# Zhongxu-Wang/ArtSpeech

Hardware: AMD Instinct MI355X
Metric: mel frames/sec (whole job; per-GPU = value / n_gpus), acoustic-model inference path, batch 32 x 200-frame utterances (higher is better)
Workload: dtype f32 (f16x3 split-operand MFMA, fp32 accumulate)

## Files before the change

### artspeech_amd/csrc/elementwise.hip

```cpp
#include "common.h"
#include <algorithm>
#include <cstring>
#include "artspeech_hip.h"
#include "conv_gemm.h"
#define AS_FILE_CLS AS_CLS_OTHER

static __device__ __forceinline__ float wave_sum(float v)
{
#pragma unroll
    for (int o = 32; o > 0; o >>= 1) v += __shfl_xor(v, o);
    return v;
}

static __device__ __forceinline__ float lrelu02(float v) { return v > 0.f ? v : 0.2f * v; }

__global__ void make_meta_kernel(const int* __restrict__ widths, const int* __restrict__ col_off, int B, int H,
                                 unsigned long long* __restrict__ meta, unsigned* __restrict__ status)
{
    const int b = blockIdx.y;
    const int W = widths[b];
    const int base = col_off[b];
    if (W > AS_META_MAX_W) {
        if (blockIdx.x == 0 && threadIdx.x == 0) as_status_raise(status, AS_STATUS_BAD_LAYOUT);
        return;
// ... 359 lines not shown
        return AS_EINVAL;
    if (N == 0) return AS_OK;
    const size_t wsz = (size_t)MM * K * sizeof(float);
    AsProfScope prof__(AS_FILE_CLS, 2.0 * M * K * (double)N, 4.0 * (K + M) * (double)N, s);
    const dim3 grid(as_cdiv(N, 64)), block(256);
    if (M == 1) hipLaunchKernelGGL(project_cols_kernel<1>, grid, block, wsz, s, x, ldx, K, N, w, bias, M, y, ldy, pros, ld_pros, col_off, B, track0);
    else if (M <= 4) hipLaunchKernelGGL(project_cols_kernel<4>, grid, block, wsz, s, x, ldx, K, N, w, bias, M, y, ldy, pros, ld_pros, col_off, B, track0);
    else hipLaunchKernelGGL(project_cols_kernel<16>, grid, block, wsz, s, x, ldx, K, N, w, bias, M, y, ldy, pros, ld_pros, col_off, B, track0);
    AS_CHECK_LAUNCH();
    return AS_OK;
}

__global__ void __launch_bounds__(256)
pointwise_small_kernel(const float* __restrict__ x, int ldx, int K, int N, const float* __restrict__ w, const float* __restrict__ bias, int M,
                       float* y1, int ld1, u32x4_t* h1, float* y2, int ld2, u32x4_t* h2)
{
    const int j = blockIdx.x * 256 + threadIdx.x, g = blockIdx.y;
    if (j > N) return;
    float xv[16];
#pragma unroll
    for (int k = 0; k < 16; ++k) xv[k] = (k < K && j < N) ? x[(size_t)k * ldx + j] : 0.f;
    float v[8];
#pragma unroll
    for (int r = 0; r < 8; ++r) {
        const int m = 8 * g + r, mm = m < M ? m : M - 1;
        float acc = bias ? bias[mm] : 0.f;
#pragma unroll
        for (int k = 0; k < 16; ++k)
            if (k < K) acc = __builtin_fmaf(w[(size_t)mm * K + k], xv[k], acc);
        const bool ok = m < M && j < N;
        v[r] = ok ? acc : 0.f;
        if (ok && y1) y1[(size_t)m * ld1 + j] = acc;
        if (ok && y2) y2[(size_t)m * ld2 + j] = acc;
    }
    u32x4_t h, l;
    split2(v, h, l);
    const size_t NX = (size_t)N + 1, at = ((size_t)(g >> 1) * 4 + (g & 1)) * NX + j;
    if (h1) { h1[at] = h; h1[at + 2 * NX] = l; }
    if (h2) { h2[at] = h; h2[at + 2 * NX] = l; }
}

extern "C" int as_pointwise_small_f32(const float* x, int ldx, int K, int N, const float* w, const float* bias, int M, float* y1, int ld1,
                                      uint16_t* yh1, float* y2, int ld2, uint16_t* yh2, as_stream_t stream)
{
    if (!x || !w || K <= 0 || K > 16 || M <= 0 || N < 0 || ldx < N || (!y1 && !yh1 && !y2 && !yh2) || (y1 && ld1 < N) || (y2 && ld2 < N)) return AS_EINVAL;
    if (((reinterpret_cast<uintptr_t>(yh1) | reinterpret_cast<uintptr_t>(yh2)) & 15) != 0) return AS_EINVAL;
    if (N == 0) return AS_OK;
    const int groups = (yh1 || yh2) ? 2 * as_kbx(M) : (M + 7) / 8;
    AsProfScope prof__(AS_FILE_CLS, 2.0 * M * K * (double)N, 4.0 * (K + 2.0 * M * ((y1 || yh1 ? 1 : 0) + (y2 || yh2 ? 1 : 0))) * (double)N, (hipStream_t)stream);
    hipLaunchKernelGGL(pointwise_small_kernel, dim3(as_cdiv(N + 1, 256), groups), dim3(256), 0, (hipStream_t)stream, x, ldx, K, N, w, bias, M, y1, ld1,
                       reinterpret_cast<u32x4_t*>(yh1), y2, ld2, reinterpret_cast<u32x4_t*>(yh2));
    AS_CHECK_LAUNCH();
    return AS_OK;
}

__global__ void __launch_bounds__(1024)
durations_kernel(const float* __restrict__ dur_f, const int* __restrict__ forced, const int* __restrict__ tok_off,
                 int B, int* __restrict__ dur_i, int* __restrict__ frame_off, int* __restrict__ tok_of_frame,
                 int max_frames, unsigned* __restrict__ status, const float* __restrict__ pros, int ldr)
{
    __shared__ int sums[1024];
    const int ntok = tok_off[B];
    const int t = threadIdx.x;
    const int per = (ntok + 1023) / 1024, lo = min(t * per, ntok), hi = min(lo + per, ntok);
    int ub = 0;
    if (pros && lo < hi) {
        int l = 0, h = B - 1;
        while (h > l) {
            const int mid = (l + h + 1) >> 1;
            if (tok_off[mid] <= lo) l = mid;
            else h = mid - 1;
        }
        ub = l;
    }
    int local = 0;
    for (int i = lo; i < hi; ++i) {
        int d;
        if (forced) d = forced[i];
        else {
            float v = dur_f[i];
            if (pros) {
                while (ub + 1 < B && tok_off[ub + 1] <= i) ++ub;
                v = v * pros[(size_t)ub * ldr + AS_PROSODY_DUR];
            }
            const bool fin = fabsf(v) <= 3.0e38f;
            if (!fin) as_status_raise(status, AS_STATUS_F16_RANGE);
            const float r = fin ? rintf(v) : 1.f;
            d = (int)(r < 1.f ? 1.f : fminf(r, 16384.f));
        }
        dur_i[i] = d;
        local += d;
    }
    sums[t] = local;
    __syncthreads();
    for (int off = 1; off < 1024; off <<= 1) {
        const int v = t >= off ? sums[t - off] : 0;
        __syncthreads();
        sums[t] += v;
        __syncthreads();
    }
    int f = sums[t] - local;
    if (t == 0) frame_off[B] = sums[1023];
    int b = 0;
    if (lo < hi || ntok == 0) {
        for (b = 0; b < B; ++b) {
            const int first = tok_off[b];
            if (first >= lo && first < hi) {
                int fb = f;
                for (int i = lo; i < first; ++i) fb += dur_i[i];
                frame_off[b] = fb;
            }
        }
    }
    if (t == 0)
        for (b = 0; b < B; ++b)
            if (tok_off[b] >= ntok) frame_off[b] = sums[1023];
    if (!tok_of_frame) return;
    for (int i = lo; i < hi; ++i) {
        const int d = dur_i[i];
        for (int r = 0; r < d; ++r, ++f)
            if (f < max_frames) tok_of_frame[f] = i;
    }
}

int as_durations_prosody_launch(const float* dur_f32, const int32_t* forced_dur, const int32_t* tok_off, int B, const float* pros, int ld_pros,
                                int32_t* dur_i32, int32_t* frame_off, int32_t* tok_of_frame, int max_frames, hipStream_t stream)
{
    if ((!dur_f32 && !forced_dur) || !tok_off || !dur_i32 || !frame_off || B < 0 || B > 1024) return AS_EINVAL;
    if (pros && (forced_dur || B < 1 || ld_pros < AS_PROSODY_DIM)) return AS_EINVAL;
    AsProfScope prof__(AS_FILE_CLS, 0, 0, stream);
    hipLaunchKernelGGL(durations_kernel, dim3(1), dim3(1024), 0, stream, dur_f32, forced_dur, tok_off, B,
                       dur_i32, frame_off, tok_of_frame, max_frames, as_status_words_device(), pros, ld_pros);
    AS_CHECK_LAUNCH();
    return AS_OK;
}

extern "C" int as_durations_f32(const float* dur_f32, const int32_t* forced_dur, const int32_t* tok_off, int B,
                                int32_t* dur_i32, int32_t* frame_off, int32_t* tok_of_frame, int max_frames,
                                as_stream_t stream)
{
    return as_durations_prosody_launch(dur_f32, forced_dur, tok_off, B, nullptr, 0, dur_i32, frame_off, tok_of_frame, max_frames,
                                       (hipStream_t)stream);
}

__global__ void expand_kernel(const float* __restrict__ x, int ldx, int C, const int* __restrict__ tok_of_frame,
                              int n_frames, int rep, float* __restrict__ y, int ldy)
{
    const int j = blockIdx.x * blockDim.x + threadIdx.x;
    const int c = blockIdx.y;
    if (j >= n_frames * rep) return;
    y[(size_t)c * ldy + j] = x[(size_t)c * ldx + tok_of_frame[j / rep]];
}

extern "C" int as_expand_f32(const float* x, int ldx, int C, const int32_t* tok_of_frame, int n_frames, int repeat,
                             float* y, int ldy, as_stream_t stream)
{
    if (!x || !y || !tok_of_frame || C <= 0 || n_frames < 0 || repeat < 1 || ldy < n_frames * repeat) return AS_EINVAL;
    if (n_frames == 0) return AS_OK;
    AsProfScope prof__(AS_FILE_CLS, 0, 0, (hipStream_t)stream);
    hipLaunchKernelGGL(expand_kernel, dim3(as_cdiv((long)n_frames * repeat, 256), C), dim3(256), 0, (hipStream_t)stream,
                       x, ldx, C, tok_of_frame, n_frames, repeat, y, ldy);
    AS_CHECK_LAUNCH();
    return AS_OK;
}

__global__ void __launch_bounds__(256)
ref_features_kernel(const float* __restrict__ mel, int ldm, int n_mels, const float* __restrict__ f0_raw,
                    const float* __restrict__ ema_raw, int lde, int N, const float* __restrict__ stats,
                    float* __restrict__ feat, int ldf)
{
    __shared__ float part[8][32];
    const int col = threadIdx.x & 31, sl = threadIdx.x >> 5;
    const int j = blockIdx.x * 32 + col;
    const int jc = j < N ? j : N - 1;
    constexpr int RMAX = 16;
    float v[RMAX];
#pragma unroll
    for (int r = 0; r < RMAX; ++r) {
        const int m = sl + 8 * r;
        v[r] = mel[(size_t)(m < n_mels ? m : 0) * ldm + jc];
    }
    float ss = 0.f;
#pragma unroll
    for (int r = 0; r < RMAX; ++r) {
        if (sl + 8 * r < n_mels) {
            const float e = expf(v[r] * 4.0f + -4.0f);
            ss += e * e;
        }
    }
    for (int m = sl + 8 * RMAX; m < n_mels; m += 8) {
        const float e = expf(mel[(size_t)m * ldm + jc] * 4.0f + -4.0f);
        ss += e * e;
    }
    part[sl][col] = ss;
    __syncthreads();
    if (j >= N) return;
    if (sl == 0) {
        float tot = 0.f;
#pragma unroll
        for (int q = 0; q < 8; ++q) tot += part[q][col];
        feat[j] = (logf(sqrtf(tot)) - stats[0]) / stats[1];
    } else if (sl == 1) {
        feat[(size_t)ldf + j] = (f0_raw[j] - stats[2]) / stats[3];
    } else {
        for (int c = sl - 2; c < 10; c += 6) feat[(size_t)(2 + c) * ldf + j] = (ema_raw[(size_t)c * lde + j] - stats[4 + c]) / stats[14 + c];
    }
}

extern "C" int as_ref_features_f32(const float* mel, int ldm, int n_mels, const float* f0_raw, const float* ema_raw,
                                   int lde, int N, const float* stats24, float* feat, int ldf, as_stream_t stream)
{
    if (!mel || !f0_raw || !ema_raw || !stats24 || !feat || N < 0 || n_mels <= 0 || ldm < N || lde < N || ldf < N) return AS_EINVAL;
    if (N == 0) return AS_OK;
    AsProfScope prof__(AS_FILE_CLS, 0, 0, (hipStream_t)stream);
    hipLaunchKernelGGL(ref_features_kernel, dim3(as_cdiv(N, 32)), dim3(256), 0, (hipStream_t)stream, mel, ldm, n_mels,
                       f0_raw, ema_raw, lde, N, stats24, feat, ldf);
    AS_CHECK_LAUNCH();
    return AS_OK;
}

__global__ void crop_kernel(const float* __restrict__ src, int lds, const int* __restrict__ src_off, int start,
                            float* __restrict__ dst, int ldd, const int* __restrict__ dst_off, int C)
{
    const int b = blockIdx.y, c = blockIdx.z;
    const int L = dst_off[b + 1] - dst_off[b];
    for (int i = blockIdx.x * blockDim.x + threadIdx.x; i < L; i += gridDim.x * blockDim.x)
        dst[(size_t)c * ldd + dst_off[b] + i] = src[(size_t)c * lds + src_off[b] + start + i];
}

extern "C" int as_crop_f32(const float* src, int lds, const int32_t* src_off, int start, float* dst, int ldd,
                           const int32_t* dst_off, int B, int C, int max_len, as_stream_t stream)
{
    if (!src || !dst || !src_off || !dst_off || B < 0 || C <= 0) return AS_EINVAL;
    if (B == 0 || max_len <= 0) return AS_OK;
    AsProfScope prof__(AS_FILE_CLS, 0, 0, (hipStream_t)stream);
    hipLaunchKernelGGL(crop_kernel, dim3(as_cdiv(max_len, 256), B, C), dim3(256), 0, (hipStream_t)stream, src, lds,
                       src_off, start, dst, ldd, dst_off, C);
    AS_CHECK_LAUNCH();
    return AS_OK;
}

__global__ void rows_to_images_kernel(const float* __restrict__ src, int lds, const int* __restrict__ src_off, int start,
                                      float* __restrict__ dst, const int* __restrict__ img_off, int H)
{
    const int b = blockIdx.y, h = blockIdx.z;
    const int Wb = (img_off[b + 1] - img_off[b]) / H;
    for (int i = blockIdx.x * blockDim.x + threadIdx.x; i < Wb; i += gridDim.x * blockDim.x)
        dst[(size_t)img_off[b] + (size_t)h * Wb + i] = src[(size_t)h * lds + src_off[b] + start + i];
}

extern "C" int as_rows_to_images_f32(const float* src, int lds, const int32_t* src_off, int start, int H, float* dst,
                                     const int32_t* img_off, int B, int max_w, as_stream_t stream)
{
    if (!src || !dst || !src_off || !img_off || B < 0 || H <= 0) return AS_EINVAL;
    if (B == 0 || max_w <= 0) return AS_OK;
    AsProfScope prof__(AS_FILE_CLS, 0, 0, (hipStream_t)stream);
    hipLaunchKernelGGL(rows_to_images_kernel, dim3(as_cdiv(max_w, 256), B, H), dim3(256), 0, (hipStream_t)stream, src, lds,
                       src_off, start, dst, img_off, H);
    AS_CHECK_LAUNCH();
    return AS_OK;
}

__global__ void bn_lrelu_maxpool_rows_kernel(const float* __restrict__ x, int ldx, const int* __restrict__ tok_off, int H, int k,
                                             const float* __restrict__ scale, const float* __restrict__ shift, float slope,
                                             float* __restrict__ y, int ldy, int to_channels)
{
    const int b = blockIdx.y, c = blockIdx.z;
    const int t0 = tok_off[b], Wb = tok_off[b + 1] - t0, Hout = H / k;
    const float* xr = x + (size_t)c * ldx + (size_t)H * t0;
    const float sc = scale[c], sh = shift[c];
    for (int i = blockIdx.x * blockDim.x + threadIdx.x; i < Hout * Wb; i += gridDim.x * blockDim.x) {
        const int ho = i / Wb, w = i - ho * Wb;
        float m = -INFINITY;
        for (int r = 0; r < k; ++r) {
            float v = xr[(size_t)(ho * k + r) * Wb + w] * sc + sh;
            v = v > 0.f ? v : slope * v;
            m = fmaxf(m, v);
        }
        if (to_channels) y[(size_t)(c * Hout + ho) * ldy + t0 + w] = m;
        else y[(size_t)c * ldy + (size_t)Hout * t0 + i] = m;
    }
}

extern "C" int as_bn_lrelu_maxpool_rows_f32(const float* x, int ldx, const int32_t* tok_off, int B, int C, int H, int k,
                                            const float* scale, const float* shift, float slope, float* y, int ldy,
                                            int to_channels, int total_frames, as_stream_t stream)
{
    if (!x || !y || !tok_off || !scale || !shift || B < 0 || C <= 0 || H <= 0 || k <= 0 || k > H) return AS_EINVAL;
    if (B == 0 || total_frames <= 0) return AS_OK;
    AsProfScope prof__(AS_FILE_CLS, 0, 4.0 * C * (double)total_frames * (H + H / k), (hipStream_t)stream);
    const int per_utt = as_cdiv((long)(H / k) * total_frames, B);
    int gx = as_cdiv(per_utt, 256);
    gx = gx < 1 ? 1 : gx > 64 ? 64 : gx;
    hipLaunchKernelGGL(bn_lrelu_maxpool_rows_kernel, dim3(gx, B, C), dim3(256), 0, (hipStream_t)stream, x, ldx, tok_off, H, k, scale,
                       shift, slope, y, ldy, to_channels);
    AS_CHECK_LAUNCH();
    return AS_OK;
}

typedef float f32x2u __attribute__((ext_vector_type(2), aligned(4)));
template <int KH>
static __device__ __forceinline__ void dwconv_down_body(const AsDownArgs& a, int b, int g, int bx, int gxn)
{
    __shared__ float ws[8][KH * 3 + 1];
    const float* __restrict__ x = a.x;
    const int ldx = a.ldx, Hin = a.Hin, ldy = a.ldy, Hout = a.Hout, C = a.C, Nout = a.n_out, act = a.lrelu;
    const int* __restrict__ in_off = a.in_off;
    const int* __restrict__ in_w = a.in_w;
    const int* __restrict__ out_off = a.out_off;
    const int* __restrict__ out_w = a.out_w;
    const float* __restrict__ w = a.w;
    const float* __restrict__ bias = a.bias;
    float* __restrict__ y = a.y;
    u32x4_t* __restrict__ yh = reinterpret_cast<u32x4_t*>(a.yh);
    const int sh = KH == 3 ? 2 : 1, ph = KH == 3 ? 1 : 0;
    const int c0 = g * 8;
    const int Wi = in_w[b], Wo = out_w[b];
    const size_t NX = (size_t)Nout + 1, plane = ((size_t)(g >> 1) * 4 + (g & 1)) * NX;
    if (yh && b == 0 && bx == 0 && threadIdx.x < 2) yh[plane + (size_t)threadIdx.x * 2 * NX + Nout] = u32x4_t{0u, 0u, 0u, 0u};
    if (threadIdx.x < 8 * (KH * 3 + 1)) {
        const int r = threadIdx.x / (KH * 3 + 1), k = threadIdx.x % (KH * 3 + 1), c = c0 + r;
        ws[r][k] = c < C ? (k < KH * 3 ? w[(size_t)c * KH * 3 + k] : bias[c]) : 0.f;
    }
    __syncthreads();
    const int ib = in_off[b], ob = out_off[b], lane = threadIdx.x & 63;
    for (int i0 = bx * 256; i0 < Hout * Wo; i0 += gxn * 256) {
        const int i = i0 + threadIdx.x, ic = min(i, Hout * Wo - 1);
        const int ho = ic / Wo, wo = ic - ho * Wo;
        const bool has_r = 2 * wo + 1 < Wi;
        const int pc = Wi >= 2 ? (has_r ? 2 * wo : 2 * wo - 1) : 0;
        const bool own_left = lane == 0 && wo > 0;
        float t[8];
#pragma unroll
        for (int r = 0; r < 8; ++r) t[r] = 0.f;
        f32x2u p2[8][KH];
        float lo[8][KH];
        bool okh[KH];
        int base[KH];
#pragma unroll
        for (int a = 0; a < KH; ++a) {
            const int hi = ho * sh - ph + a, hc = min(max(hi, 0), Hin - 1);
            okh[a] = hi >= 0 && hi < Hin;
            base[a] = ib + hc * Wi;
        }
        if (Wi >= 2) {
#pragma unroll
            for (int a = 0; a < KH; ++a)
#pragma unroll
                for (int r = 0; r < 8; ++r) p2[r][a] = *reinterpret_cast<const f32x2u*>(x + (size_t)min(c0 + r, C - 1) * ldx + base[a] + pc);
        } else {
#pragma unroll
            for (int a = 0; a < KH; ++a)
#pragma unroll
                for (int r = 0; r < 8; ++r) { const float e = x[(size_t)min(c0 + r, C - 1) * ldx + base[a]]; p2[r][a] = f32x2u{e, e}; }
        }
        if (own_left) {
#pragma unroll
            for (int a = 0; a < KH; ++a)
#pragma unroll
                for (int r = 0; r < 8; ++r) lo[r][a] = x[(size_t)min(c0 + r, C - 1) * ldx + base[a] + 2 * wo - 1];
        }
        float v[8][KH][3];
#pragma unroll
        for (int a = 0; a < KH; ++a)
#pragma unroll
            for (int r = 0; r < 8; ++r) {
                const float x0 = (has_r || Wi < 2) ? p2[r][a].x : p2[r][a].y, x1 = p2[r][a].y;
                const float xl = __shfl_up(x1, 1);
                v[r][a][0] = own_left ? lo[r][a] : xl; v[r][a][1] = x0; v[r][a][2] = x1;
            }
#pragma unroll
        for (int r = 0; r < 8; ++r) {
            float s = 0.f;
#pragma unroll
            for (int a = 0; a < KH; ++a) {
                if (okh[a] && wo > 0) s += v[r][a][0] * ws[r][a * 3 + 0];
                if (okh[a]) s += v[r][a][1] * ws[r][a * 3 + 1];
                if (okh[a] && has_r) s += v[r][a][2] * ws[r][a * 3 + 2];
            }
            s += ws[r][KH * 3];
            if (act) s = lrelu02(s);
            if (c0 + r >= C) s = 0.f;
            else if (y && i < Hout * Wo) y[(size_t)(c0 + r) * ldy + ob + i] = s;
            t[r] = s;
        }
        if (yh && i < Hout * Wo) {
            u32x4_t h, l;
            split2(t, h, l);
            const size_t at = plane + ob + i;
            yh[at] = h;
            yh[at + 2 * NX] = l;
        }
    }
}

static int down_one(const AsDownArgs& a, hipStream_t stream);

static int dwconv_launch(const float* x, int ldx, const int32_t* in_off, const int32_t* in_w, int Hin, float* y, int ldy, const int32_t* out_off,
                         const int32_t* out_w, int Hout, const float* w, const float* bias, int kh, int B, int C, int max_out, int lrelu,
                         uint16_t* yh, int Nout, hipStream_t stream)
{
    AsDownArgs a;
    memset(&a, 0, sizeof(a));
    a.kind = 0; a.x = x; a.ldx = ldx; a.in_off = in_off; a.in_w = in_w; a.Hin = Hin; a.y = y; a.ldy = ldy; a.out_off = out_off; a.out_w = out_w;
    a.Hout = Hout; a.w = w; a.bias = bias; a.kh = kh; a.B = B; a.C = C; a.max_out = max_out; a.lrelu = lrelu; a.yh = yh; a.n_out = Nout;
    return down_one(a, stream);
}

extern "C" int as_dwconv_down_f32(const float* x, int ldx, const int32_t* in_off, const int32_t* in_w, int Hin,
                                  float* y, int ldy, const int32_t* out_off, const int32_t* out_w, int Hout,
                                  const float* w, const float* bias, int kh, int B, int C, int max_out, int lrelu,
                                  as_stream_t stream)
{
    return dwconv_launch(x, ldx, in_off, in_w, Hin, y, ldy, out_off, out_w, Hout, w, bias, kh, B, C, max_out, lrelu, nullptr, 0, (hipStream_t)stream);
}

extern "C" int as_dwconv_down_image_f32(const float* x, int ldx, const int32_t* in_off, const int32_t* in_w, int Hin, const int32_t* out_off,
                                        const int32_t* out_w, int Hout, const float* w, const float* bias, int kh, int B, int C, int max_out,
                                        int lrelu, uint16_t* yh, int n_out, as_stream_t stream)
{
    if (!yh) return AS_EINVAL;
    return dwconv_launch(x, ldx, in_off, in_w, Hin, nullptr, 0, out_off, out_w, Hout, w, bias, kh, B, C, max_out, lrelu, yh, n_out, (hipStream_t)stream);
}

template <int PH>
static __device__ __forceinline__ void avgpool_down_body(const AsDownArgs& a, int b, int g, int bx, int gxn)
{
    const float* __restrict__ x = a.x;
    const int ldx = a.ldx, ldy = a.ldy, Hout = a.Hout, C = a.C, Nout = a.n_out, yh_lrelu = a.lrelu, ldr = a.ldr;
    const int* __restrict__ in_off = a.in_off;
    const int* __restrict__ in_w = a.in_w;
    const int* __restrict__ out_off = a.out_off;
    const int* __restrict__ out_w = a.out_w;
    const float* __restrict__ res = a.res;
    float* __restrict__ y = a.y;
    u32x4_t* __restrict__ yh = reinterpret_cast<u32x4_t*>(a.yh);
    const int c0 = g * 8;
    const int Wi = in_w[b], Wo = out_w[b], ib = in_off[b], ob = out_off[b];
    const size_t NX = (size_t)Nout + 1, plane = ((size_t)(g >> 1) * 4 + (g & 1)) * NX;
    if (yh && b == 0 && bx == 0 && threadIdx.x < 2) yh[plane + (size_t)threadIdx.x * 2 * NX + Nout] = u32x4_t{0u, 0u, 0u, 0u};
    for (int i = bx * 256 + threadIdx.x; i < Hout * Wo; i += gxn * 256) {
        const int ho = i / Wo, wo = i - ho * Wo;
        const bool has_r = 2 * wo + 1 < Wi;
        const int pc = Wi >= 2 ? (has_r ? 2 * wo : 2 * wo - 1) : 0;
        f32x2u p2[8][PH];
        float rv[8];
#pragma unroll
        for (int r = 0; r < 8; ++r) {
            const float* xr = x + (size_t)min(c0 + r, C - 1) * ldx + ib;
#pragma unroll
            for (int a = 0; a < PH; ++a) {
                if (Wi >= 2) p2[r][a] = *reinterpret_cast<const f32x2u*>(xr + (size_t)(ho * PH + a) * Wi + pc);
                else { const float e = xr[(size_t)(ho * PH + a) * Wi]; p2[r][a] = f32x2u{e, e}; }
            }
            rv[r] = res ? res[(size_t)min(c0 + r, C - 1) * ldr + ob + i] : 0.f;
        }
        float t[8];
#pragma unroll
        for (int r = 0; r < 8; ++r) {
            float s = 0.f;
#pragma unroll
            for (int a = 0; a < PH; ++a) {
                s += (has_r || Wi < 2) ? p2[r][a].x : p2[r][a].y;
                s += p2[r][a].y;
            }
            s = s / (float)(2 * PH);
            if (res) s = (s + rv[r]) / 1.41421356237309504880f;
            if (c0 + r < C) {
                if (y) y[(size_t)(c0 + r) * ldy + ob + i] = s;
                if (yh_lrelu) s = lrelu02(s);
            } else {
                s = 0.f;
            }
            t[r] = s;
        }
        if (yh) {
            u32x4_t h, l;
            split2(t, h, l);
            const size_t at = plane + ob + i;
            yh[at] = h;
            yh[at + 2 * NX] = l;
        }
    }
}

static int avgpool_launch(const float* x, int ldx, const int32_t* in_off, const int32_t* in_w, int Hin, float* y, int ldy, const int32_t* out_off,
                          const int32_t* out_w, int Hout, int pool_h, const float* res, int ldr, int B, int C, int max_out, uint16_t* yh, int Nout,
                          int yh_lrelu, hipStream_t stream)
{
    AsDownArgs a;
    memset(&a, 0, sizeof(a));
    a.kind = 1; a.x = x; a.ldx = ldx; a.in_off = in_off; a.in_w = in_w; a.Hin = Hin; a.y = y; a.ldy = ldy; a.out_off = out_off; a.out_w = out_w;
    a.Hout = Hout; a.pool_h = pool_h; a.res = res; a.ldr = ldr; a.B = B; a.C = C; a.max_out = max_out; a.yh = yh; a.n_out = Nout; a.lrelu = yh_lrelu;
    return down_one(a, stream);
}

extern "C" int as_avgpool_down_f32(const float* x, int ldx, const int32_t* in_off, const int32_t* in_w, int Hin,
                                   float* y, int ldy, const int32_t* out_off, const int32_t* out_w, int Hout,
                                   int pool_h, const float* res, int ldr, int B, int C, int max_out, as_stream_t stream)
{
    if (!y) return AS_EINVAL;
    return avgpool_launch(x, ldx, in_off, in_w, Hin, y, ldy, out_off, out_w, Hout, pool_h, res, ldr, B, C, max_out, nullptr, 0, 0, (hipStream_t)stream);
}

extern "C" int as_avgpool_down_image_f32(const float* x, int ldx, const int32_t* in_off, const int32_t* in_w, int Hin, float* y, int ldy,
                                         const int32_t* out_off, const int32_t* out_w, int Hout, int pool_h, const float* res, int ldr, int B,
                                         int C, int max_out, uint16_t* yh, int n_out, int yh_lrelu, as_stream_t stream)
{
    if (!yh) return AS_EINVAL;
    return avgpool_launch(x, ldx, in_off, in_w, Hin, y, ldy, out_off, out_w, Hout, pool_h, res, ldr, B, C, max_out, yh, n_out, yh_lrelu,
                          (hipStream_t)stream);
}

static __device__ __forceinline__ void stem_pool_image_body(const AsDownArgs& a, int b, int g, int bx, int gxn)
{
    __shared__ float ws[8][10];
    const float* __restrict__ x = a.x;
    const int Hin = a.Hin, Hout = a.Hout, ph = a.pool_h, Kp = a.Kp, KH = a.kh, C = a.C, Nout = a.n_out;
    const int* __restrict__ in_off = a.in_off;
    const int* __restrict__ in_w = a.in_w;
    const int* __restrict__ out_off = a.out_off;
    const int* __restrict__ out_w = a.out_w;
    const float* __restrict__ w = a.w;
    const float* __restrict__ bias = a.bias;
    u32x4_t* __restrict__ yh = reinterpret_cast<u32x4_t*>(a.yh);
    const int c0 = g * 8;
    const int Wi = in_w[b], Wo = out_w[b];
    const size_t NX = (size_t)Nout + 1, plane = ((size_t)(g >> 1) * 4 + (g & 1)) * NX;
    if (b == 0 && bx == 0 && threadIdx.x < 2) yh[plane + (size_t)threadIdx.x * 2 * NX + Nout] = u32x4_t{0u, 0u, 0u, 0u};
    if (threadIdx.x < 80) {
        const int r = threadIdx.x / 10, k = threadIdx.x % 10, c = c0 + r;
        ws[r][k] = c < C ? (k < 9 ? (k < KH * 3 ? w[(size_t)k * Kp * C + c] : 0.f) : (bias ? bias[c] : 0.f)) : 0.f;
    }
    __syncthreads();
    const int ib = in_off[b], ob = out_off[b], pad = KH / 2;
    for (int i = bx * 256 + threadIdx.x; i < Hout * Wo; i += gxn * 256) {
        const int ho = i / Wo, wo = i - ho * Wo;
        float win[4][4];
#pragma unroll
        for (int r = 0; r < 4; ++r) {
            const int hi = ho * ph - pad + r, hc = min(max(hi, 0), Hin - 1);
#pragma unroll
            for (int cc = 0; cc < 4; ++cc) {
                const int wi = 2 * wo - 1 + cc, wc = min(max(wi, 0), Wi - 1);
                win[r][cc] = x[ib + hc * Wi + wc];
            }
        }
#pragma unroll
        for (int r = 0; r < 4; ++r) {
            const int hi = ho * ph - pad + r;
#pragma unroll
            for (int cc = 0; cc < 4; ++cc) {
                const int wi = 2 * wo - 1 + cc;
                const bool ok = r < ph + KH - 1 && hi >= 0 && hi < Hin && wi >= 0 && wi < Wi;
                win[r][cc] = ok ? win[r][cc] : 0.f;
            }
        }
        const bool dup = 2 * wo + 1 >= Wi;
        float t[8];
#pragma unroll
        for (int r = 0; r < 8; ++r) {
            float wr[10];
#pragma unroll
            for (int k = 0; k < 10; ++k) wr[k] = ws[r][k];
            float s = 0.f;
#pragma unroll
            for (int a = 0; a < 2; ++a) {
                if (a >= ph) break;
                float v[2];
#pragma unroll
                for (int cc = 0; cc < 2; ++cc) {
                    float sum = 0.f;
#pragma unroll
                    for (int ta = 0; ta < 3; ++ta) {
                        if (ta >= KH) break;
#pragma unroll
                        for (int td = 0; td < 3; ++td) sum += wr[ta * 3 + td] * win[a + ta][cc + td];
                    }
                    v[cc] = sum + wr[9];
                }
                s += v[0];
                s += dup ? v[0] : v[1];
            }
            t[r] = c0 + r < C ? s / (float)(2 * ph) : 0.f;
        }
        u32x4_t h, l;
        split2(t, h, l);
        const size_t at = plane + ob + i;
        yh[at] = h;
        yh[at + 2 * NX] = l;
    }
}

extern "C" int as_stem_pool_image_f32(const float* x, const int32_t* in_off, const int32_t* in_w, int Hin, const int32_t* out_off,
                                      const int32_t* out_w, int Hout, int pool_h, const float* w, int Kp, const float* bias, int kh, int B, int C,
                                      int max_out, uint16_t* yh, int n_out, as_stream_t stream)
{
    AsDownArgs a;
    memset(&a, 0, sizeof(a));
    a.kind = 2; a.x = x; a.in_off = in_off; a.in_w = in_w; a.Hin = Hin; a.out_off = out_off; a.out_w = out_w; a.Hout = Hout; a.pool_h = pool_h;
    a.w = w; a.Kp = Kp; a.bias = bias; a.kh = kh; a.B = B; a.C = C; a.max_out = max_out; a.yh = yh; a.n_out = n_out;
    return down_one(a, (hipStream_t)stream);
}

#define DOWN_MAXP 6
struct DownMulti {
    int32_t n, pad_;
    int32_t blk0[DOWN_MAXP + 2];
    int32_t gx[DOWN_MAXP], gz[DOWN_MAXP];
    AsDownArgs a[DOWN_MAXP];
};
template <bool HEAVY>
__global__ void __launch_bounds__(256)
down_multi_kernel(const DownMulti dm)
{
    int pi = 0;
#pragma unroll
    for (int i = 1; i < DOWN_MAXP; ++i) pi += (i < dm.n && (int)blockIdx.x >= dm.blk0[i]) ? 1 : 0;
    const AsDownArgs& a = dm.a[pi];
    const int gxn = dm.gx[pi], local = (int)blockIdx.x - dm.blk0[pi];
    const int bx = local % gxn, rest = local / gxn, b = rest % a.B, g = rest / a.B;
    if (a.kind == 0) {
        if (a.kh == 3) { if constexpr (HEAVY) dwconv_down_body<3>(a, b, g, bx, gxn); }
        else dwconv_down_body<1>(a, b, g, bx, gxn);
    } else if (a.kind == 1) {
        if (a.pool_h == 2) avgpool_down_body<2>(a, b, g, bx, gxn);
        else avgpool_down_body<1>(a, b, g, bx, gxn);
    } else {
        if constexpr (HEAVY) stem_pool_image_body(a, b, g, bx, gxn);
    }
}

static int down_check(const AsDownArgs& a)
{
    if (!a.x || !a.in_off || !a.in_w || !a.out_off || !a.out_w || a.B < 0 || a.C <= 0) return AS_EINVAL;
    if (a.yh && ((reinterpret_cast<uintptr_t>(a.yh) & 15) != 0 || a.n_out < 0)) return AS_EINVAL;
    if (a.kind == 0) return ((!a.y && !a.yh) || !a.w || !a.bias || (a.kh != 1 && a.kh != 3)) ? AS_EINVAL : AS_OK;
    if (a.kind == 1) return ((!a.y && !a.yh) || (a.pool_h != 1 && a.pool_h != 2)) ? AS_EINVAL : AS_OK;
    if (a.kind == 2) return (!a.w || !a.yh || (a.pool_h != 1 && a.pool_h != 2) || (a.kh != 1 && a.kh != 3) || a.Kp <= 0) ? AS_EINVAL : AS_OK;
    return AS_EINVAL;
}

extern "C" int as_down_multi_f32(const AsDownArgs* list_host, int n, as_stream_t stream_)
{
    static_assert(DOWN_MAXP == AS_MAX_MULTI, "header and kernel disagree");
    if (!list_host || n < 1 || n > DOWN_MAXP) return AS_EINVAL;
    DownMulti dm;
    memset(&dm, 0, sizeof(dm));
    bool heavy = false;
    for (int i = 0; i < n; ++i) {
        const AsDownArgs& a = list_host[i];
        const int r = down_check(a);
        if (r != AS_OK) return r;
        if (a.B == 0 || a.max_out <= 0) continue;
        heavy = heavy || a.kind == 2 || (a.kind == 0 && a.kh == 3);
        dm.a[dm.n] = a;
        dm.gx[dm.n] = std::min(32, as_cdiv(a.max_out, 256));
        dm.gz[dm.n] = a.yh ? 2 * as_kbx(a.C) : as_cdiv(a.C, 8);
        dm.blk0[dm.n + 1] = dm.blk0[dm.n] + dm.gx[dm.n] * a.B * dm.gz[dm.n];
        ++dm.n;
    }
    if (dm.n == 0) return AS_OK;
    AsProfScope prof__(AS_FILE_CLS, 0, 0, (hipStream_t)stream_);
    if (heavy) hipLaunchKernelGGL(down_multi_kernel<true>, dim3(dm.blk0[dm.n]), dim3(256), 0, (hipStream_t)stream_, dm);
    else hipLaunchKernelGGL(down_multi_kernel<false>, dim3(dm.blk0[dm.n]), dim3(256), 0, (hipStream_t)stream_, dm);
    AS_CHECK_LAUNCH();
    return AS_OK;
}

static int down_one(const AsDownArgs& a, hipStream_t stream) { return as_down_multi_f32(&a, 1, stream); }

__global__ void __launch_bounds__(256)
im2col_valid_kernel(const float* __restrict__ x, int ldx, const int* __restrict__ in_off, const int* __restrict__ in_w,
                    int Hin, float* __restrict__ col, int ldc, const int* __restrict__ out_off,
                    const int* __restrict__ out_w, int Hout, int K, int stride, int act, int B)
{
    const int ck = blockIdx.x;
    const int c = ck / (K * K), a = (ck / K) % K, d = ck % K;
    const int total = out_off[B];
    for (int j = threadIdx.x; j < total; j += blockDim.x) {
        int b = 0;
        while (b + 1 < B && out_off[b + 1] <= j) ++b;
        const int i = j - out_off[b], Wo = out_w[b], Wi = in_w[b];
        const int ho = i / Wo, wo = i - ho * Wo;
        float v = x[(size_t)c * ldx + in_off[b] + (size_t)(ho * stride + a) * Wi + wo * stride + d];
        if (act) v = lrelu02(v);
        col[(size_t)ck * ldc + j] = v;
    }
}

extern "C" int as_im2col_valid_f32(const float* x, int ldx, const int32_t* in_off, const int32_t* in_w, int Hin,
                                   float* col, int ldc, const int32_t* out_off, const int32_t* out_w, int Hout, int K,
                                   int stride, int lrelu, int B, int C, int max_out, as_stream_t stream)
{
    if (!x || !col || !in_off || !in_w || !out_off || !out_w || K <= 0 || stride <= 0 || B < 0 || C <= 0) return AS_EINVAL;
    if (B == 0 || max_out <= 0) return AS_OK;
    AsProfScope prof__(AS_FILE_CLS, 0, 0, (hipStream_t)stream);
    hipLaunchKernelGGL(im2col_valid_kernel, dim3(C * K * K), dim3(256), 0, (hipStream_t)stream, x, ldx, in_off, in_w, Hin, col,
                       ldc, out_off, out_w, Hout, K, stride, lrelu, B);
    AS_CHECK_LAUNCH();
    return AS_OK;
}

__global__ void __launch_bounds__(256)
im2col_valid_image_kernel(const float* __restrict__ x, int ldx, const int* __restrict__ in_off, const int* __restrict__ in_w,
                          const int* __restrict__ out_off, const int* __restrict__ out_w, int K, int stride, int act, int B, int rows,
                          u32x4_t* __restrict__ yh)
{
    const int g = blockIdx.x;
    const int total = out_off[B];
    const size_t NX = (size_t)total + 1, plane = ((size_t)(g >> 1) * 4 + (g & 1)) * NX;
    if (threadIdx.x < 2) yh[plane + (size_t)threadIdx.x * 2 * NX + total] = u32x4_t{0u, 0u, 0u, 0u};
    for (int j = threadIdx.x; j < total; j += blockDim.x) {
        int b = 0;
        while (b + 1 < B && out_off[b + 1] <= j) ++b;
        const int i = j - out_off[b], Wo = out_w[b], Wi = in_w[b];
        const int ho = i / Wo, wo = i - ho * Wo;
        float t[8];
#pragma unroll
        for (int r = 0; r < 8; ++r) {
            const int ck = g * 8 + r;
            float v = 0.f;
            if (ck < rows) {
                const int c = ck / (K * K), a = (ck / K) % K, d = ck % K;
                v = x[(size_t)c * ldx + in_off[b] + (size_t)(ho * stride + a) * Wi + wo * stride + d];
                if (act) v = lrelu02(v);
            }
            t[r] = v;
        }
        u32x4_t h, l;
        split2(t, h, l);
        yh[plane + j] = h;
        yh[plane + j + 2 * NX] = l;
    }
}

extern "C" int as_im2col_valid_image_f32(const float* x, int ldx, const int32_t* in_off, const int32_t* in_w, const int32_t* out_off,
                                         const int32_t* out_w, int K, int stride, int lrelu, int B, int C, uint16_t* yh, as_stream_t stream)
{
    if (!x || !yh || !in_off || !in_w || !out_off || !out_w || K <= 0 || stride <= 0 || B <= 0 || C <= 0 ||
        (reinterpret_cast<uintptr_t>(yh) & 15) != 0)
        return AS_EINVAL;
    AsProfScope prof__(AS_FILE_CLS, 0, 0, (hipStream_t)stream);
    hipLaunchKernelGGL(im2col_valid_image_kernel, dim3(2 * as_kbx(C * K * K)), dim3(256), 0, (hipStream_t)stream, x, ldx, in_off, in_w, out_off,
                       out_w, K, stride, lrelu, B, C * K * K, reinterpret_cast<u32x4_t*>(yh));
    AS_CHECK_LAUNCH();
    return AS_OK;
}

__global__ void __launch_bounds__(256)
mean_pool_kernel(const float* __restrict__ x, int ldx, const int* __restrict__ col_off, int B, int C, int act,
                 float* __restrict__ y, int ldy)
{
    const int lane = threadIdx.x & 63;
    const int row = blockIdx.x * 4 + (threadIdx.x >> 6);
    if (row >= C * B) return;
    const int c = row / B, b = row - c * B;
    const int o0 = col_off[b], L = col_off[b + 1] - o0;
    float s = 0.f;
    for (int i = lane; i < L; i += 64) {
        float v = x[(size_t)c * ldx + o0 + i];
        if (act) v = lrelu02(v);
        s += v;
    }
    s = wave_sum(s);
    if (lane == 0) y[(size_t)b * ldy + c] = s / (float)L;
}

extern "C" int as_mean_pool_f32(const float* x, int ldx, const int32_t* col_off, int B, int C, int lrelu, float* y,
                                int ldy, as_stream_t stream)
{
    if (!x || !y || !col_off || B < 0 || C <= 0 || ldy < C) return AS_EINVAL;
    if (B == 0) return AS_OK;
    AsProfScope prof__(AS_FILE_CLS, 0, 0, (hipStream_t)stream);
    hipLaunchKernelGGL(mean_pool_kernel, dim3(as_cdiv((long)C * B, 4)), dim3(256), 0, (hipStream_t)stream, x, ldx, col_off,
                       B, C, lrelu, y, ldy);
    AS_CHECK_LAUNCH();
    return AS_OK;
}

__global__ void __launch_bounds__(256)
dyn_geometry_kernel(const AsDynGeo g)
{
    const int z = blockIdx.z, b = blockIdx.y, B = g.B, cap1 = g.cap1;
    const int total_raw = g.frame_off[B];
    if (z == 8) {
        if (b == 0) {
            if (g.tof)
                for (int f = max(total_raw, 0) + (int)(blockIdx.x * blockDim.x + threadIdx.x); f < cap1; f += gridDim.x * blockDim.x) g.tof[f] = 0;
            if (blockIdx.x == 0 && threadIdx.x == 0 && total_raw > cap1) as_status_raise(g.status, AS_STATUS_CAPACITY);
        }
        if (blockIdx.x == 0 && threadIdx.x == 0) {
            int s = 0;
            while (s + 1 < g.n_seg && b >= g.seg_first[s + 1]) ++s;
            const int first = g.seg_first[s], o_first = min(g.frame_off[first], cap1);
            int32_t* fo = g.seg_frame_off[s];
            if (fo) fo[b - first] = min(g.frame_off[b], cap1) - o_first;
            if (b + 1 == g.seg_first[s + 1]) {
                const int len = min(g.frame_off[b + 1], cap1) - o_first;
                if (fo) fo[b + 1 - first] = len;
                if (len > g.seg_cap[s]) as_status_raise(g.status, AS_STATUS_CAPACITY);
            }
        }
        return;
    }
    const int li = z == 0 ? 0 : (z == 1 ? 1 : (z < 5 ? 2 : 3));
    const int grp = z < 2 ? 0 : (z < 5 ? z - 2 : z - 5);
    const int sc = (li == 1 || li == 3) ? 2 : 1;
    const int o = min(g.frame_off[b], cap1), e = min(g.frame_off[b + 1], cap1);
    const int W = sc * (e - o), base = grp * sc * cap1 + sc * o, u = grp * B + b;
    if (blockIdx.x == 0 && threadIdx.x == 0) {
        if (g.w[li]) g.w[li][u] = W;
        if (g.off[li]) {
            g.off[li][u] = base;
            if (b == B - 1 && (li < 2 || grp == 2)) g.off[li][u + 1] = base + W;
        }
        if (li == 2 && g.src3) g.src3[u] = o;
        if (b == 0 && grp == 0 && g.nvalid[li]) *g.nvalid[li] = sc * min(max(total_raw, 0), cap1);
    }
    unsigned long long* meta = g.meta[li];
    if (!meta) return;
    for (int i = blockIdx.x * blockDim.x + threadIdx.x; i < W; i += gridDim.x * blockDim.x)
        meta[base + i] = AS_META_PACK(0ull, (unsigned long long)i, 1ull, (unsigned long long)W);
}

int as_dyn_geometry_launch(const AsDynGeo& g, hipStream_t stream)
{
    if (!g.frame_off || g.B < 1 || g.B > 1024 || g.cap1 < 1 || g.n_seg < 1 || g.n_seg > 16) return AS_EINVAL;
    AsProfScope prof__(AS_FILE_CLS, 0, 0, stream);
    const int gx = std::min(64, std::max(1, as_cdiv(as_cdiv(2L * g.cap1, g.B), 256)));
    hipLaunchKernelGGL(dyn_geometry_kernel, dim3(gx, g.B, 9), dim3(256), 0, stream, g);
    AS_CHECK_LAUNCH();
    return AS_OK;
}

__global__ void __launch_bounds__(256)
seg_scatter_kernel(const AsSegScatter a)
{
    const int s = blockIdx.z, r = blockIdx.y;
    const int first = a.seg_first[s], last = a.seg_first[s + 1];
    const int o = 2 * a.frame_off[first], n = min(2 * (a.frame_off[last] - a.frame_off[first]), 2 * a.seg_cap[s]);
    const float* src = a.src + (size_t)r * a.ld_src + o;
    float* dst = a.dst[s] + (size_t)r * a.ld_dst[s];
    for (int i = blockIdx.x * blockDim.x + threadIdx.x; i < n; i += gridDim.x * blockDim.x) dst[i] = src[i];
}

int as_seg_scatter_launch(const AsSegScatter& a, hipStream_t stream)
{
    if (!a.src || !a.frame_off || a.rows < 1 || a.n_seg < 1 || a.n_seg > 16) return AS_EINVAL;
    AsProfScope prof__(AS_FILE_CLS, 0, 0, stream);
    int cap = 1;
    for (int s = 0; s < a.n_seg; ++s) cap = std::max(cap, 2 * a.seg_cap[s]);
    hipLaunchKernelGGL(seg_scatter_kernel, dim3(std::min(64, as_cdiv(cap, 256)), a.rows, a.n_seg), dim3(256), 0, stream, a);
    AS_CHECK_LAUNCH();
    return AS_OK;
}
```

Baseline: 1.732 million.

## Split dwconv channels across thread pairs, use buffer loads, precombine stem weights

The depthwise downsample conv now has each pair of threads share one output position, with each thread handling 4 of the 8 channels. Loads go through raw buffer loads with scalar offsets, and the fp16 split outputs are written as 64-bit halves. The stem pool kernel precomputes combined pooled-conv weights in shared memory, so each output becomes a 4x4 dot product instead of nested conv-plus-pool loops. The grid-x sizing changes from a divisor of 256 to 1024, which gives fewer blocks and more loop iterations per block. This risks lower occupancy and adds a 4GB limit check on buffer resource size.

New measurement: 1.755 million, median of 6. About the same (+1.3%).

```diff
diff --git a/artspeech_amd/csrc/elementwise.hip b/artspeech_amd/csrc/elementwise.hip
--- a/artspeech_amd/csrc/elementwise.hip
+++ b/artspeech_amd/csrc/elementwise.hip
@@ -685,6 +685,8 @@
 template <int KH>
 static __device__ __forceinline__ void dwconv_down_body(const AsDownArgs& a, int b, int g, int bx, int gxn)
 {
+    constexpr int CPT = 4, P = 2;
+    constexpr int NPOS = 256 / P;
     __shared__ float ws[8][KH * 3 + 1];
     const float* __restrict__ x = a.x;
     const int ldx = a.ldx, Hin = a.Hin, ldy = a.ldy, Hout = a.Hout, C = a.C, Nout = a.n_out, act = a.lrelu;
@@ -707,17 +709,17 @@
     }
     __syncthreads();
     const int ib = in_off[b], ob = out_off[b], lane = threadIdx.x & 63;
-    for (int i0 = bx * 256; i0 < Hout * Wo; i0 += gxn * 256) {
-        const int i = i0 + threadIdx.x, ic = min(i, Hout * Wo - 1);
+    const int q = threadIdx.x % P, cq = q * CPT;
+    const __amdgpu_buffer_rsrc_t rsX = __builtin_amdgcn_make_buffer_rsrc(const_cast<float*>(x), 0, (int)((unsigned)C * (unsigned)ldx * 4u), 0x00020000);
+    for (int i0 = bx * NPOS; i0 < Hout * Wo; i0 += gxn * NPOS) {
+        const int i = i0 + (int)threadIdx.x / P, ic = min(i, Hout * Wo - 1);
         const int ho = ic / Wo, wo = ic - ho * Wo;
         const bool has_r = 2 * wo + 1 < Wi;
         const int pc = Wi >= 2 ? (has_r ? 2 * wo : 2 * wo - 1) : 0;
-        const bool own_left = lane == 0 && wo > 0;
-        float t[8];
-#pragma unroll
-        for (int r = 0; r < 8; ++r) t[r] = 0.f;
-        f32x2u p2[8][KH];
-        float lo[8][KH];
+        const bool own_left = lane < P && wo > 0;
+        float t[CPT];
+        f32x2u p2[CPT][KH];
+        float lo[CPT][KH];
         bool okh[KH];
         int base[KH];
 #pragma unroll
@@ -726,53 +728,64 @@
             okh[a] = hi >= 0 && hi < Hin;
             base[a] = ib + hc * Wi;
         }
+        const bool full = c0 + 8 <= C;
+        auto off = [&](int r, int col) -> unsigned { return (unsigned)((full ? cq * ldx : min(c0 + cq + r, C - 1) * ldx) + col) * 4u; };
+        auto soff = [&](int r) -> int { return full ? (int)((unsigned)(c0 + r) * (unsigned)ldx * 4u) : 0; };
         if (Wi >= 2) {
 #pragma unroll
             for (int a = 0; a < KH; ++a)
 #pragma unroll
-                for (int r = 0; r < 8; ++r) p2[r][a] = *reinterpret_cast<const f32x2u*>(x + (size_t)min(c0 + r, C - 1) * ldx + base[a] + pc);
+                for (int r = 0; r < CPT; ++r) p2[r][a] = __builtin_bit_cast(f32x2u, __builtin_amdgcn_raw_buffer_load_b64(rsX, off(r, base[a] + pc), soff(r), 0));
         } else {
 #pragma unroll
             for (int a = 0; a < KH; ++a)
 #pragma unroll
-                for (int r = 0; r < 8; ++r) { const float e = x[(size_t)min(c0 + r, C - 1) * ldx + base[a]]; p2[r][a] = f32x2u{e, e}; }
+                for (int r = 0; r < CPT; ++r) { const float e = buf_load1(rsX, off(r, base[a]), soff(r)); p2[r][a] = f32x2u{e, e}; }
         }
         if (own_left) {
 #pragma unroll
             for (int a = 0; a < KH; ++a)
 #pragma unroll
-                for (int r = 0; r < 8; ++r) lo[r][a] = x[(size_t)min(c0 + r, C - 1) * ldx + base[a] + 2 * wo - 1];
-        }
-        float v[8][KH][3];
+                for (int r = 0; r < CPT; ++r) lo[r][a] = buf_load1(rsX, off(r, base[a] + 2 * wo - 1), soff(r));
+        }
+        float v[CPT][KH][3];
 #pragma unroll
         for (int a = 0; a < KH; ++a)
 #pragma unroll
-            for (int r = 0; r < 8; ++r) {
+            for (int r = 0; r < CPT; ++r) {
                 const float x0 = (has_r || Wi < 2) ? p2[r][a].x : p2[r][a].y, x1 = p2[r][a].y;
-                const float xl = __shfl_up(x1, 1);
+                const float xl = __shfl_up(x1, P);
                 v[r][a][0] = own_left ? lo[r][a] : xl; v[r][a][1] = x0; v[r][a][2] = x1;
             }
 #pragma unroll
-        for (int r = 0; r < 8; ++r) {
+        for (int r = 0; r < CPT; ++r) {
+            const int c = c0 + cq + r;
             float s = 0.f;
 #pragma unroll
             for (int a = 0; a < KH; ++a) {
-                if (okh[a] && wo > 0) s += v[r][a][0] * ws[r][a * 3 + 0];
-                if (okh[a]) s += v[r][a][1] * ws[r][a * 3 + 1];
-                if (okh[a] && has_r) s += v[r][a][2] * ws[r][a * 3 + 2];
-            }
-            s += ws[r][KH * 3];
+                if (okh[a] && wo > 0) s += v[r][a][0] * ws[cq + r][a * 3 + 0];
+                if (okh[a]) s += v[r][a][1] * ws[cq + r][a * 3 + 1];
+                if (okh[a] && has_r) s += v[r][a][2] * ws[cq + r][a * 3 + 2];
+            }
+            s += ws[cq + r][KH * 3];
             if (act) s = lrelu02(s);
-            if (c0 + r >= C) s = 0.f;
-            else if (y && i < Hout * Wo) y[(size_t)(c0 + r) * ldy + ob + i] = s;
+            if (c >= C) s = 0.f;
+            else if (y && i < Hout * Wo) y[(size_t)c * ldy + ob + i] = s;
             t[r] = s;
         }
         if (yh && i < Hout * Wo) {
-            u32x4_t h, l;
-            split2(t, h, l);
             const size_t at = plane + ob + i;
-            yh[at] = h;
-            yh[at + 2 * NX] = l;
+            u32x2_t h, l;
+#pragma unroll
+            for (int e = 0; e < CPT / 2; ++e) {
+                unsigned hu, lu;
+                split2_pair(t[2 * e], t[2 * e + 1], hu, lu);
+                h[e] = hu;
+                l[e] = lu;
+            }
+            u32x2_t* yh2 = reinterpret_cast<u32x2_t*>(yh);
+            yh2[2 * at + q] = h;
+            yh2[2 * (at + 2 * NX) + q] = l;
         }
     }
 }
@@ -898,6 +911,7 @@
 static __device__ __forceinline__ void stem_pool_image_body(const AsDownArgs& a, int b, int g, int bx, int gxn)
 {
     __shared__ float ws[8][10];
+    __shared__ __attribute__((aligned(16))) float wc[8][2][16];
     const float* __restrict__ x = a.x;
     const int Hin = a.Hin, Hout = a.Hout, ph = a.pool_h, Kp = a.Kp, KH = a.kh, C = a.C, Nout = a.n_out;
     const int* __restrict__ in_off = a.in_off;
@@ -916,7 +930,19 @@
         ws[r][k] = c < C ? (k < 9 ? (k < KH * 3 ? w[(size_t)k * Kp * C + c] : 0.f) : (bias ? bias[c] : 0.f)) : 0.f;
     }
     __syncthreads();
+    {
+        const int r = threadIdx.x >> 5, dup = (threadIdx.x >> 4) & 1, rr = (threadIdx.x >> 2) & 3, cw = threadIdx.x & 3;
+        float sum = 0.f;
+        for (int pa = 0; pa < ph; ++pa)
+            for (int ta = 0; ta < KH; ++ta)
+                for (int cc = 0; cc < 2; ++cc)
+                    for (int td = 0; td < 3; ++td)
+                        if (pa + ta == rr && (dup ? td : cc + td) == cw) sum += ws[r][ta * 3 + td];
+        wc[r][dup][rr * 4 + cw] = sum;
+    }
+    __syncthreads();
     const int ib = in_off[b], ob = out_off[b], pad = KH / 2;
+    const float bsc = (float)(2 * ph);
     for (int i = bx * 256 + threadIdx.x; i < Hout * Wo; i += gxn * 256) {
         const int ho = i / Wo, wo = i - ho * Wo;
         float win[4][4];
@@ -925,8 +951,8 @@
             const int hi = ho * ph - pad + r, hc = min(max(hi, 0), Hin - 1);
 #pragma unroll
             for (int cc = 0; cc < 4; ++cc) {
-                const int wi = 2 * wo - 1 + cc, wc = min(max(wi, 0), Wi - 1);
-                win[r][cc] = x[ib + hc * Wi + wc];
+                const int wi = 2 * wo - 1 + cc, wc_ = min(max(wi, 0), Wi - 1);
+                win[r][cc] = x[ib + hc * Wi + wc_];
             }
         }
 #pragma unroll
@@ -939,33 +965,18 @@
                 win[r][cc] = ok ? win[r][cc] : 0.f;
             }
         }
-        const bool dup = 2 * wo + 1 >= Wi;
+        const int dup = 2 * wo + 1 >= Wi ? 1 : 0;
         float t[8];
 #pragma unroll
         for (int r = 0; r < 8; ++r) {
-            float wr[10];
-#pragma unroll
-            for (int k = 0; k < 10; ++k) wr[k] = ws[r][k];
-            float s = 0.f;
-#pragma unroll
-            for (int a = 0; a < 2; ++a) {
-                if (a >= ph) break;
-                float v[2];
-#pragma unroll
-                for (int cc = 0; cc < 2; ++cc) {
-                    float sum = 0.f;
-#pragma unroll
-                    for (int ta = 0; ta < 3; ++ta) {
-                        if (ta >= KH) break;
-#pragma unroll
-                        for (int td = 0; td < 3; ++td) sum += wr[ta * 3 + td] * win[a + ta][cc + td];
-                    }
-                    v[cc] = sum + wr[9];
-                }
-                s += v[0];
-                s += dup ? v[0] : v[1];
-            }
-            t[r] = c0 + r < C ? s / (float)(2 * ph) : 0.f;
+            float s = bsc * ws[r][9];
+#pragma unroll
+            for (int q = 0; q < 4; ++q) {
+                const f32x4 k4 = *reinterpret_cast<const f32x4*>(&wc[r][dup][q * 4]);
+#pragma unroll
+                for (int e = 0; e < 4; ++e) s += k4[e] * win[q][e];
+            }
+            t[r] = c0 + r < C ? s / bsc : 0.f;
         }
         u32x4_t h, l;
         split2(t, h, l);
@@ -1018,7 +1029,7 @@
 {
     if (!a.x || !a.in_off || !a.in_w || !a.out_off || !a.out_w || a.B < 0 || a.C <= 0) return AS_EINVAL;
     if (a.yh && ((reinterpret_cast<uintptr_t>(a.yh) & 15) != 0 || a.n_out < 0)) return AS_EINVAL;
-    if (a.kind == 0) return ((!a.y && !a.yh) || !a.w || !a.bias || (a.kh != 1 && a.kh != 3)) ? AS_EINVAL : AS_OK;
+    if (a.kind == 0) return ((!a.y && !a.yh) || !a.w || !a.bias || (a.kh != 1 && a.kh != 3) || (double)a.C * a.ldx * 4.0 >= 4294967296.0) ? AS_EINVAL : AS_OK;
     if (a.kind == 1) return ((!a.y && !a.yh) || (a.pool_h != 1 && a.pool_h != 2)) ? AS_EINVAL : AS_OK;
     if (a.kind == 2) return (!a.w || !a.yh || (a.pool_h != 1 && a.pool_h != 2) || (a.kh != 1 && a.kh != 3) || a.Kp <= 0) ? AS_EINVAL : AS_OK;
     return AS_EINVAL;
@@ -1038,7 +1049,7 @@
         if (a.B == 0 || a.max_out <= 0) continue;
         heavy = heavy || a.kind == 2 || (a.kind == 0 && a.kh == 3);
         dm.a[dm.n] = a;
-        dm.gx[dm.n] = std::min(32, as_cdiv(a.max_out, 256));
+        dm.gx[dm.n] = std::min(32, as_cdiv(a.max_out, 1024));
         dm.gz[dm.n] = a.yh ? 2 * as_kbx(a.C) : as_cdiv(a.C, 8);
         dm.blk0[dm.n + 1] = dm.blk0[dm.n] + dm.gx[dm.n] * a.B * dm.gz[dm.n];
         ++dm.n;
```
